# CPJKU/audio_sheet_retrieval

Hardware: AMD Instinct MI355X
Metric: snippet-pairs/sec embedded+ranked (32-d CCA) (higher is better)
Workload: dtype f32

## Files before the change

audio_sheet_retrieval_amd/csrc/conv_wino4_kernels.hip:

```cpp
#include <hip/hip_runtime.h>
#include <stdint.h>
#include <stdlib.h>
#include <algorithm>
#include <type_traits>
#include <vector>
#include "asr_kernels.h"
#include "repack_elems.inl"
#include "wino4_epilogue.h"

#ifndef ASR_WINO4_ABL
#define ASR_WINO4_ABL 0
#endif

namespace asr {

typedef float floatx4q __attribute__((ext_vector_type(4)));
typedef float float2q __attribute__((ext_vector_type(2)));
typedef unsigned uint2q __attribute__((ext_vector_type(2)));

struct Wino4Args {
    const float *in, *wpk, *bnp;
    float *out;
    int N, H, W, OH, OW;
    int ty_img, tx_img;
    int coutp;
    int tiles;
    int total;
    double *stats;
    int epi;
};

__device__ __forceinline__ float elu_fastq(float y) { return y > 0.0f ? y : __expf(y) - 1.0f; }

__device__ __forceinline__ floatx4q bn_elu4q(floatx4q x, float mean, float scale, float beta) {
    const floatx4q y = (x - floatx4q{mean, mean, mean, mean}) * floatx4q{scale, scale, scale, scale} +
                       floatx4q{beta, beta, beta, beta};
    return floatx4q{elu_fastq(y[0]), elu_fastq(y[1]), elu_fastq(y[2]), elu_fastq(y[3])};
}
typedef int int4q __attribute__((ext_vector_type(4)));
__device__ __forceinline__ void buffer_store_q(float v, unsigned voff, int4q rsrc, unsigned soff) {
    asm volatile("buffer_store_dword %0, %1, %2, %3 offen" ::"v"(v), "v"(voff), "s"(rsrc), "s"(soff) : "memory");
}

template <typename T> __device__ __forceinline__ T splatq(float c);
template <> __device__ __forceinline__ float2q splatq<float2q>(float c) { return float2q{c, c}; }
template <> __device__ __forceinline__ floatx4q splatq<floatx4q>(float c) { return floatx4q{c, c, c, c}; }
template <typename T> __device__ __forceinline__ T fmaq(float c, T x, T y) {
    return __builtin_elementwise_fma(splatq<T>(c), x, y);
}

template <typename T> __device__ __forceinline__ void in6(T &d0, T &d1, T &d2, T &d3, T &d4, T &d5) {
    const T r0 = fmaq(4.f, d0, fmaq(-5.f, d2, d4));
    const T t1 = fmaq(-4.f, d2, d4), t2 = fmaq(-4.f, d1, d3);
    const T t3 = d4 - d2, t4 = d3 - d1;
    const T r5 = fmaq(4.f, d1, fmaq(-5.f, d3, d5));
    d0 = r0; d1 = t1 + t2; d2 = t1 - t2; d3 = fmaq(2.f, t4, t3); d4 = fmaq(-2.f, t4, t3); d5 = r5;
}
template <typename T> __device__ __forceinline__ void out6(T m0, T m1, T m2, T m3, T m4, T m5, T &y0, T &y1, T &y2, T &y3) {
    const T s1 = m1 + m2, s2 = m1 - m2, s3 = m3 + m4, s4 = m3 - m4;
    y0 = (m0 + s1) + s3;
    y1 = fmaq(2.f, s4, s2);
    y2 = fmaq(4.f, s3, s1);
    y3 = fmaq(8.f, s4, s2) + m5;
}

template <int CIN, int COUT, bool POOL, int WAVES, bool RAW>
__global__ __launch_bounds__(64 * WAVES, 1) void conv3x3_wino4g(Wino4Args a) {
    constexpr int KS = CIN / 4, NB = CIN / 8, T = 64 * WAVES;
    constexpr int WS = 16;
    constexpr int WD = 6;
    constexpr int WQ = 72;
    static_assert(CIN % 8 == 0, "channel blocks of 8");
    extern __shared__ __align__(16) float w_lds[];
    const int tid = threadIdx.x, lane = tid & 63;
    const int wave = __builtin_amdgcn_readfirstlane(tid >> 6);
    const int nt0 = blockIdx.y;
    for (int i = tid; i < KS * 36 * 4 * 16; i += T) {
        const int row = i >> 4, nn = i & 15;
        const int gg = row & 3, kp = row >> 2, ks = kp / 36, p = kp - ks * 36;
        const int qq = (ks & 1) * 36 + p;
        w_lds[i] = a.wpk[((((size_t)(ks >> 1) * 18 + (qq >> 2)) * 4 + gg) * a.coutp + nt0 * 16 + nn) * 4 + (qq & 3)];
    }
    __syncthreads();

    const int m = lane & 15, g = lane >> 4, n = lane & 15;
    const float *w_lane = w_lds + g * WS + n;
    const int chn = nt0 * 16 + n;
    const bool ch_ok = chn < COUT;
    const float bmean = (!RAW && ch_ok) ? a.bnp[chn] : 0.f;
    const float bscale = (!RAW && ch_ok) ? a.bnp[a.coutp + chn] : 1.f;
    const float bbeta = (!RAW && ch_ok) ? a.bnp[2 * a.coutp + chn] : 0.f;
    const int per_img = a.ty_img * a.tx_img;

    for (int mt = blockIdx.x * WAVES + wave; mt < a.total; mt += gridDim.x * WAVES) {
        const int tnum = mt * 16 + m;
        const bool tvalid = tnum < a.tiles;
        const int tcl = min(tnum, a.tiles - 1);
        const int img = tcl / per_img;
        const int trest = tcl - img * per_img;
        const int tty = trest / a.tx_img, ttx = trest - tty * a.tx_img;
        const int py = 4 * tty, px = 4 * ttx;
        const float *ibase = a.in + (int64_t)img * a.H * a.W * CIN + 2 * g;
        int rowb[6], colb[6];
        unsigned oy_m = 0, ox_m = 0;
#pragma unroll
        for (int i = 0; i < 6; ++i) {
            const int y = py - 1 + i, x = px - 1 + i;
            oy_m |= (unsigned)(y >= 0 && y < a.H) << i;
            ox_m |= (unsigned)(x >= 0 && x < a.W) << i;
            rowb[i] = min(max(y, 0), a.H - 1) * a.W * CIN;
            colb[i] = min(max(x, 0), a.W - 1) * CIN;
        }
        if (!tvalid) oy_m = 0;
        const bool interior = __builtin_amdgcn_ballot_w64(oy_m != 0x3fu || ox_m != 0x3fu) == 0;
        unsigned my_off;
        int my_ext;
        if (POOL) {
            my_off = (((unsigned)img * a.OH + 2 * tty) * a.OW + 2 * ttx) * COUT;
            const int nr = min(2, a.OH - 2 * tty), nc = min(2, a.OW - 2 * ttx);
            my_ext = (tvalid && nr > 0 && nc > 0) ? (nr | (nc << 8)) : 0;
        } else {
            my_off = (((unsigned)img * a.H + py) * a.W + px) * COUT;
            const int nr = min(4, a.H - py), nc = min(4, a.W - px);
            my_ext = tvalid ? (nr | (nc << 8)) : 0;
        }

        floatx4q acc[36];
#pragma unroll
        for (int p = 0; p < 36; ++p) acc[p] = floatx4q{0.f, 0.f, 0.f, 0.f};

        float2q nxt[6][6];
#pragma unroll
        for (int i = 0; i < 6; ++i)
#pragma unroll
            for (int j = 0; j < 6; ++j) nxt[i][j] = *reinterpret_cast<const float2q *>(ibase + rowb[i] + colb[j]);
        float wpre[WD];
#pragma unroll
        for (int q = 0; q < WD; ++q) wpre[q] = w_lane[q * 4 * WS];
#pragma unroll 1
        for (int t = 0; t < NB; ++t) {
            float2q dp[6][6];
            if (interior) {
#pragma unroll
                for (int i = 0; i < 6; ++i)
#pragma unroll
                    for (int j = 0; j < 6; ++j) dp[i][j] = nxt[i][j];
            } else {
#pragma unroll
                for (int i = 0; i < 6; ++i)
#pragma unroll
                    for (int j = 0; j < 6; ++j)
                        dp[i][j] = (((oy_m >> i) & (ox_m >> j)) & 1u) ? nxt[i][j] : float2q{0.f, 0.f};
            }
            if (t + 1 < NB && !(ASR_WINO4_ABL & 2)) {
#pragma unroll
                for (int i = 0; i < 6; ++i)
#pragma unroll
                    for (int j = 0; j < 6; ++j)
                        nxt[i][j] = *reinterpret_cast<const float2q *>(ibase + rowb[i] + colb[j] + 8 * (t + 1));
            }
#pragma unroll
            for (int j = 0; j < 6; ++j) in6(dp[0][j], dp[1][j], dp[2][j], dp[3][j], dp[4][j], dp[5][j]);
#pragma unroll
            for (int i = 0; i < 6; ++i) in6(dp[i][0], dp[i][1], dp[i][2], dp[i][3], dp[i][4], dp[i][5]);
            const float *wk = w_lane + (2 * t) * (36 * 4 * WS);
            const float *wn = (t + 1 < NB) ? wk + 2 * 36 * 4 * WS : w_lane;
            float wv[WQ + WD];
#pragma unroll
            for (int q = 0; q < WD; ++q) wv[q] = wpre[q];
#pragma unroll
            for (int q0 = 0; q0 < WQ; q0 += 2) {
#pragma unroll
                for (int q = q0; q < q0 + 2; ++q)
                    wv[q + WD] = (q + WD < WQ) ? wk[(q + WD) * 4 * WS] : wn[(q + WD - WQ) * 4 * WS];
                __builtin_amdgcn_sched_barrier(0);
#pragma unroll
                for (int q = q0; q < q0 + 2; ++q) {
                    const int c = q / 36, p = q % 36;
                    acc[p] = __builtin_amdgcn_mfma_f32_16x16x4f32(dp[p / 6][p % 6][c], wv[q], acc[p], 0, 0, 0);
                }
                __builtin_amdgcn_sched_barrier(0);
            }
#pragma unroll
            for (int q = 0; q < WD; ++q) wpre[q] = wv[WQ + q];
        }

        unsigned eo[4];
        int ee[4];
#pragma unroll
        for (int r = 0; r < 4; ++r) {
            eo[r] = (unsigned)__shfl((int)my_off, 4 * g + r);
            ee[r] = __shfl(my_ext, 4 * g + r);
        }
        if (!ch_ok) continue;
        floatx4q tc[4][6];
#pragma unroll
        for (int nu = 0; nu < 6; ++nu)
            out6(acc[nu], acc[6 + nu], acc[12 + nu], acc[18 + nu], acc[24 + nu], acc[30 + nu], tc[0][nu], tc[1][nu], tc[2][nu],
                 tc[3][nu]);
        if (POOL) {
#pragma unroll
            for (int pr = 0; pr < 2; ++pr) {
                floatx4q ya[4], yb[4];
                out6(tc[2 * pr][0], tc[2 * pr][1], tc[2 * pr][2], tc[2 * pr][3], tc[2 * pr][4], tc[2 * pr][5], ya[0], ya[1],
                     ya[2], ya[3]);
                out6(tc[2 * pr + 1][0], tc[2 * pr + 1][1], tc[2 * pr + 1][2], tc[2 * pr + 1][3], tc[2 * pr + 1][4],
                     tc[2 * pr + 1][5], yb[0], yb[1], yb[2], yb[3]);
#pragma unroll
                for (int pc = 0; pc < 2; ++pc) {
#pragma unroll
                    for (int r = 0; r < 4; ++r) {
                        if (pr >= (ee[r] & 0xff) || pc >= (ee[r] >> 8)) continue;
                        const float v0 = ya[2 * pc][r], v1 = ya[2 * pc + 1][r], v2 = yb[2 * pc][r], v3 = yb[2 * pc + 1][r];
                        const float hi = fmaxf(fmaxf(v0, v1), fmaxf(v2, v3));
                        const float lo = fminf(fminf(v0, v1), fminf(v2, v3));
                        const float x = bscale >= 0.0f ? hi : lo;
                        a.out[(size_t)eo[r] + (size_t)(pr * a.OW + pc) * COUT + chn] =
                            elu_fastq((x - bmean) * bscale + bbeta);
                    }
                }
            }
        } else {
#pragma unroll
            for (int i = 0; i < 4; ++i) {
                floatx4q y[4];
                out6(tc[i][0], tc[i][1], tc[i][2], tc[i][3], tc[i][4], tc[i][5], y[0], y[1], y[2], y[3]);
#pragma unroll
                for (int j = 0; j < 4; ++j) {
#pragma unroll
                    for (int r = 0; r < 4; ++r) {
                        if (i >= (ee[r] & 0xff) || j >= (ee[r] >> 8)) continue;
                        const float v = RAW ? y[j][r] : elu_fastq((y[j][r] - bmean) * bscale + bbeta);
                        a.out[(size_t)eo[r] + (size_t)(i * a.W + j) * COUT + chn] = v;
                    }
                }
            }
        }
    }
}

template <int CIN, int COUT, bool POOL, int SLICE = COUT, int PW = 1, bool RAW = false>
__global__ __launch_bounds__(64 * (PW + (SLICE + 15) / 16), 1) void conv3x3_wino4s(Wino4Args a) {
    static_assert(!(RAW && POOL), "the raw form has no pooled epilogue");
    constexpr int NT = (SLICE + 15) / 16, NB = CIN / 8, KS = CIN / 4;
    static_assert(PW == 1 || PW == 2, "one or two producer waves");
    static_assert(PW + NT <= 4, "one wave per SIMD");
    static_assert(SLICE == COUT || (SLICE % 16 == 0 && COUT % SLICE == 0), "slices are whole n-tiles");
    constexpr int VB = 36 * 16 * 8;
    static_assert(CIN % 8 == 0, "channel blocks of 8");
    extern __shared__ __align__(16) float vbuf[];
    const int tid = threadIdx.x, lane = tid & 63;
    const int wave = __builtin_amdgcn_readfirstlane(tid >> 6);
    const bool producer = wave < PW;
    const int m = lane & 15, g = lane >> 4, n = lane & 15;
    const int per_img = a.ty_img * a.tx_img;

    int mt, mt_end, mt_stride;
    if ((gridDim.x & 7) == 0) {
        const int per_x = (a.total + 7) >> 3;
        const int r0 = (int)(blockIdx.x & 7) * per_x;
        mt_end = min(r0 + per_x, a.total);
        mt_stride = (int)(gridDim.x >> 3);
        mt = r0 + (int)(blockIdx.x >> 3);
    } else {
        mt_end = a.total; mt_stride = (int)gridDim.x; mt = (int)blockIdx.x;
    }
    if (mt >= mt_end) {
        if constexpr (RAW) {
            if (a.stats)
                for (int c = threadIdx.x; c < 2 * COUT; c += blockDim.x) a.stats[(size_t)blockIdx.x * 2 * COUT + c] = 0.0;
        }
        return;
    }

    auto tile_of = [&](int mtile, int &img, int &tty, int &ttx, bool &tvalid) {
        const int tnum = mtile * 16 + m;
        tvalid = tnum < a.tiles;
        const int tcl = min(tnum, a.tiles - 1);
        img = tcl / per_img;
        const int trest = tcl - img * per_img;
        tty = trest / a.tx_img;
        ttx = trest - tty * a.tx_img;
    };
    float *vlane = vbuf + (g * 32 + 2 * m);

    if (producer) {
        unsigned poff[6][6];
        unsigned keep[6][6];
        bool interior = false;
        auto setup = [&](int mtile) {
            int img, tty, ttx;
            bool tvalid;
            tile_of(mtile, img, tty, ttx, tvalid);
            const int py = 4 * tty, px = 4 * ttx;
            const unsigned ib = ((unsigned)img * a.H * a.W * CIN + 2 * g) * 4u;
            unsigned rowb[6], colb[6];
            unsigned oy_m = 0, ox_m = 0;
#pragma unroll
            for (int i = 0; i < 6; ++i) {
                const int y = py - 1 + i, x = px - 1 + i;
                oy_m |= (unsigned)(y >= 0 && y < a.H) << i;
                ox_m |= (unsigned)(x >= 0 && x < a.W) << i;
                rowb[i] = (unsigned)(min(max(y, 0), a.H - 1) * a.W * CIN) * 4u;
                colb[i] = (unsigned)(min(max(x, 0), a.W - 1) * CIN) * 4u;
            }
            if (!tvalid) oy_m = 0;
            interior = __builtin_amdgcn_ballot_w64(oy_m != 0x3fu || ox_m != 0x3fu) == 0;
#pragma unroll
            for (int i = 0; i < 6; ++i)
#pragma unroll
                for (int j = 0; j < 6; ++j) {
                    poff[i][j] = ib + rowb[i] + colb[j];
                    keep[i][j] = 0u - (((oy_m >> i) & (ox_m >> j)) & 1u);
                }
        };
        float2q nxt[6][6];
        auto load = [&](int t) {
            const char *cb = reinterpret_cast<const char *>(a.in + 8 * t);
#pragma unroll
            for (int i = 0; i < 6; ++i)
#pragma unroll
                for (int j = 0; j < 6; ++j) nxt[i][j] = *reinterpret_cast<const float2q *>(cb + poff[i][j]);
        };
        const int n_mt = (mt_end - mt + mt_stride - 1) / mt_stride;
        const int n_steps = n_mt * NB;
        int passed = 0;
        int t = wave;
        while (t >= NB) { t -= NB; mt += mt_stride; }
        if (mt < mt_end) { setup(mt); load(t); }
        for (int step = wave; step < n_steps; step += PW) {
            constexpr int FIRST = 4;
            float2q dp[6][6];
            const bool inner = interior;
            if (inner) {
#pragma unroll
                for (int j = 0; j < 6; ++j) {
#pragma unroll
                    for (int i = 0; i < 6; ++i) dp[i][j] = nxt[i][j];
                    if (!(ASR_WINO4_ABL & 8)) in6(dp[0][j], dp[1][j], dp[2][j], dp[3][j], dp[4][j], dp[5][j]);
                }
            } else {
#pragma unroll
                for (int i = 0; i < 6; ++i)
#pragma unroll
                    for (int j = 0; j < 6; ++j)
                        dp[i][j] = __builtin_bit_cast(float2q, __builtin_bit_cast(uint2q, nxt[i][j]) & uint2q{keep[i][j], keep[i][j]});
                if (!(ASR_WINO4_ABL & 8)) {
#pragma unroll
                for (int j = 0; j < FIRST; ++j) in6(dp[0][j], dp[1][j], dp[2][j], dp[3][j], dp[4][j], dp[5][j]);
                }
            }
#pragma unroll
            for (int p = 0; p < 36; ++p) asm volatile("" : "+v"(dp[p / 6][p % 6]));
            {
                int tn = t + PW, mtn = mt;
                while (tn >= NB) { tn -= NB; mtn += mt_stride; }
                if (!(ASR_WINO4_ABL & 2) && step + PW < n_steps) {
                    if (mtn != mt) setup(mtn);
                    load(tn);
                }
                t = tn; mt = mtn;
            }
            if (!(ASR_WINO4_ABL & 8)) {
            if (!inner) {
#pragma unroll
            for (int j = FIRST; j < 6; ++j) in6(dp[0][j], dp[1][j], dp[2][j], dp[3][j], dp[4][j], dp[5][j]);
            }
#pragma unroll
            for (int i = 0; i < 6; ++i) in6(dp[i][0], dp[i][1], dp[i][2], dp[i][3], dp[i][4], dp[i][5]);
            }
            while (passed < step) { __syncthreads(); ++passed; }
            float *vb = vlane + (step & 1) * VB;
            if (!(ASR_WINO4_ABL & 16)) {
#pragma unroll
            for (int p = 0; p < 36; ++p) *reinterpret_cast<float2q *>(vb + p * 128) = dp[p / 6][p % 6];
            } else {
#pragma unroll
            for (int p = 0; p < 36; ++p) asm volatile("" ::"v"(dp[p / 6][p % 6]));
            }
            __syncthreads();
            ++passed;
        }
        while (passed < n_steps + 1) { __syncthreads(); ++passed; }
        return;
    }

    const int nt = wave - PW;
    const int chn = (int)blockIdx.y * SLICE + nt * 16 + n;
    const bool ch_ok = chn < COUT;
    float bmean = (!RAW && ch_ok) ? a.bnp[chn] : 0.f;
    float bscale = (!RAW && ch_ok) ? a.bnp[a.coutp + chn] : 1.f;
    float bbeta = (!RAW && ch_ok) ? a.bnp[2 * a.coutp + chn] : 0.f;
    double st1 = 0.0, st2 = 0.0;
    int4q orsrc;
    {
        const uint64_t obase = reinterpret_cast<uint64_t>(a.out);
        orsrc.x = (int)(uint32_t)obase;
        orsrc.y = (int)(uint32_t)(obase >> 32);
        orsrc.z = (int)((unsigned)a.N * a.OH * a.OW * COUT * 4u);
        orsrc.w = 0x00020000;
    }
    const unsigned wlane = ((unsigned)g * a.coutp + chn) * 16u;
    const float *wl = a.wpk;
    constexpr int wstep = 4 * ((COUT + 15) / 16 * 16);
    floatx4q bw[2][18];
#pragma unroll
    for (int j = 0; j < 18; ++j)
        bw[0][j] = *reinterpret_cast<const floatx4q *>(reinterpret_cast<const char *>(wl) + (size_t)j * (wstep * 16) + wlane);
    int step = 0;
    for (; mt < mt_end; mt += mt_stride) {
        unsigned my_off;
        int my_ext;
        {
            int img, tty, ttx;
            bool tvalid;
            tile_of(mt, img, tty, ttx, tvalid);
            if (POOL) my_off = (((unsigned)img * a.OH + 2 * tty) * a.OW + 2 * ttx) * COUT;
            else my_off = (((unsigned)img * a.H + 4 * tty) * a.W + 4 * ttx) * COUT;
            my_ext = wino4_extent(POOL, POOL ? a.OH : a.H, POOL ? a.OW : a.W, tty, ttx, tvalid);
        }
        int epi_mode = 0;
        if constexpr (!RAW) {
            if (a.epi)
                epi_mode = __builtin_amdgcn_ballot_w64(!wino4_rows_full(my_ext, POOL)) == 0 ? 1 : (wino4_general_form(POOL) ? 2 : 0);
        }
        unsigned voff[9];
#pragma unroll
        for (int k = 0; k < 9; ++k) {
            voff[k] = wlane + (unsigned)k * (2 * wstep * 16);
            asm volatile("" : "+v"(voff[k]));
        }
        floatx4q acc[36];
        auto reload = [&](const float *wn, auto set_c) {
            constexpr int SET = decltype(set_c)::value;
            if (ASR_WINO4_ABL & 4) return;
            const char *wnb = reinterpret_cast<const char *>(wn);
#pragma unroll
            for (int k = 0; k < 9; ++k) {
                unsigned vo = voff[k];
                asm volatile("" : "+v"(vo));
                bw[SET][2 * k] = *reinterpret_cast<const floatx4q *>(wnb + vo);
                bw[SET][2 * k + 1] = *reinterpret_cast<const floatx4q *>(wnb + (wstep * 16) + vo);
            }
        };
        auto run_step = [&](const float *vb, const float *wn, auto cur_c, auto first) {
            constexpr bool FIRST = decltype(first)::value;
            constexpr int CUR = decltype(cur_c)::value;
            using NXT = std::integral_constant<int, CUR ^ 1>;
            __syncthreads();
            reload(wn, NXT{});
            __builtin_amdgcn_sched_barrier(0);
            float2q dp[2][12];
#pragma unroll
            for (int i = 0; i < 12; ++i) dp[0][i] = *reinterpret_cast<const float2q *>(vb + i * 128);
#pragma unroll
            for (int grp = 0; grp < 3; ++grp) {
                if (grp < 2) {
#pragma unroll
                    for (int i = 0; i < 12; ++i)
                        dp[(grp + 1) & 1][i] = *reinterpret_cast<const float2q *>(vb + ((grp + 1) * 12 + i) * 128);
                }
#pragma unroll
                for (int c = 0; c < 2; ++c)
#pragma unroll
                    for (int i = 0; i < 12; ++i) {
                        const int p = grp * 12 + i;
                        if (FIRST && c == 0)
                            acc[p] = __builtin_amdgcn_mfma_f32_16x16x4f32(dp[grp & 1][i][c], bw[CUR][(c * 36 + p) >> 2][(c * 36 + p) & 3],
                                                                          floatx4q{0.f, 0.f, 0.f, 0.f}, 0, 0, 0);
                        else
                            acc[p] = __builtin_amdgcn_mfma_f32_16x16x4f32(dp[grp & 1][i][c], bw[CUR][(c * 36 + p) >> 2][(c * 36 + p) & 3], acc[p],
                                                                          0, 0,
                                                                          0);
                    }
                __builtin_amdgcn_sched_barrier(0);
            }
        };
        using C0 = std::integral_constant<int, 0>;
        using C1 = std::integral_constant<int, 1>;
        auto wblock = [&](int t) {
            unsigned blk = (unsigned)(((t + 1) % NB) * 72) * wstep;
            asm volatile("" : "+s"(blk));
            return wl + blk;
        };
        run_step(vlane + (step & 1) * VB, wblock(0), C0{}, std::true_type{});
        ++step;
#pragma unroll 1
        for (int t = 1; t + 1 < NB; t += 2) {
            run_step(vlane + (step & 1) * VB, wblock(t), C1{}, std::false_type{});
            ++step;
            run_step(vlane + (step & 1) * VB, wblock(t + 1), C0{}, std::false_type{});
            ++step;
        }
        if constexpr ((NB & 1) == 0) {
            run_step(vlane + (step & 1) * VB, wblock(NB - 1), C1{}, std::false_type{});
            ++step;
        } else {
#pragma unroll
            for (int j = 0; j < 18; ++j) bw[0][j] = bw[1][j];
        }

        unsigned eo[4];
        int ee[4];
#pragma unroll
        for (int r = 0; r < 4; ++r) {
            eo[r] = (unsigned)__shfl((int)my_off, 4 * g + r);
            ee[r] = __shfl(my_ext, 4 * g + r);
        }
        if (!ch_ok) continue;
        floatx4q tc[4][6];
#pragma unroll
        for (int nu = 0; nu < 6; ++nu)
            out6(acc[nu], acc[6 + nu], acc[12 + nu], acc[18 + nu], acc[24 + nu], acc[30 + nu], tc[0][nu], tc[1][nu], tc[2][nu],
                 tc[3][nu]);
        auto fast_epilogue = [&](auto rows_c) {
            constexpr bool ROWS = decltype(rows_c)::value;
            constexpr int SP = POOL ? 2 : 4;
            unsigned vo[4][SP];
#pragma unroll
            for (int r = 0; r < 4; ++r)
#pragma unroll
                for (int c = 0; c < SP; ++c) vo[r][c] = wino4_store_offset(eo[r], ee[r], chn, c, COUT);
#pragma unroll
            for (int i = 0; i < SP; ++i) {
                const unsigned soff = wino4_row_bytes(i, a.OW, COUT);
                floatx4q res[SP];
                if constexpr (POOL) {
                    floatx4q ya[4], yb[4];
                    out6(tc[2 * i][0], tc[2 * i][1], tc[2 * i][2], tc[2 * i][3], tc[2 * i][4], tc[2 * i][5], ya[0], ya[1], ya[2],
                         ya[3]);
                    out6(tc[2 * i + 1][0], tc[2 * i + 1][1], tc[2 * i + 1][2], tc[2 * i + 1][3], tc[2 * i + 1][4],
                         tc[2 * i + 1][5], yb[0], yb[1], yb[2], yb[3]);
#pragma unroll
                    for (int pc = 0; pc < 2; ++pc) {
                        const floatx4q hi = __builtin_elementwise_max(__builtin_elementwise_max(ya[2 * pc], ya[2 * pc + 1]),
                                                                      __builtin_elementwise_max(yb[2 * pc], yb[2 * pc + 1]));
                        const floatx4q lo = __builtin_elementwise_min(__builtin_elementwise_min(ya[2 * pc], ya[2 * pc + 1]),
                                                                      __builtin_elementwise_min(yb[2 * pc], yb[2 * pc + 1]));
                        res[pc] = bn_elu4q(bscale >= 0.0f ? hi : lo, bmean, bscale, bbeta);
                    }
                } else {
                    floatx4q y[4];
                    out6(tc[i][0], tc[i][1], tc[i][2], tc[i][3], tc[i][4], tc[i][5], y[0], y[1], y[2], y[3]);
#pragma unroll
                    for (int j = 0; j < 4; ++j) res[j] = bn_elu4q(y[j], bmean, bscale, bbeta);
                }
#pragma unroll
                for (int j = 0; j < SP; ++j)
#pragma unroll
                    for (int r = 0; r < 4; ++r) {
                        if (ASR_WINO4_ABL & 32) asm volatile("" ::"v"(res[j][r]));
                        else buffer_store_q(res[j][r], ROWS ? wino4_store_offset_row(vo[r][j], ee[r], i) : vo[r][j], orsrc, soff);
                    }
            }
        };
        if (epi_mode == 1) { fast_epilogue(std::false_type{}); continue; }
        if constexpr (!RAW && wino4_general_form(POOL)) {
            if (epi_mode == 2) { fast_epilogue(std::true_type{}); continue; }
        }
        if (POOL) {
#pragma unroll
            for (int pr = 0; pr < 2; ++pr) {
                floatx4q ya[4], yb[4];
                out6(tc[2 * pr][0], tc[2 * pr][1], tc[2 * pr][2], tc[2 * pr][3], tc[2 * pr][4], tc[2 * pr][5], ya[0], ya[1],
                     ya[2], ya[3]);
                out6(tc[2 * pr + 1][0], tc[2 * pr + 1][1], tc[2 * pr + 1][2], tc[2 * pr + 1][3], tc[2 * pr + 1][4],
                     tc[2 * pr + 1][5], yb[0], yb[1], yb[2], yb[3]);
#pragma unroll
                for (int pc = 0; pc < 2; ++pc) {
#pragma unroll
                    for (int r = 0; r < 4; ++r) {
                        if (pr >= (ee[r] & 0xff) || pc >= (ee[r] >> 8)) continue;
                        const float v0 = ya[2 * pc][r], v1 = ya[2 * pc + 1][r], v2 = yb[2 * pc][r], v3 = yb[2 * pc + 1][r];
                        const float hi = fmaxf(fmaxf(v0, v1), fmaxf(v2, v3));
                        const float lo = fminf(fminf(v0, v1), fminf(v2, v3));
                        const float x = bscale >= 0.0f ? hi : lo;
                        const float res = elu_fastq((x - bmean) * bscale + bbeta);
                        if (ASR_WINO4_ABL & 32) asm volatile("" ::"v"(res));
                        else a.out[(size_t)eo[r] + (size_t)(pr * a.OW + pc) * COUT + chn] = res;
                    }
                }
            }
        } else {
#pragma unroll
            for (int i = 0; i < 4; ++i) {
                floatx4q y[4];
                out6(tc[i][0], tc[i][1], tc[i][2], tc[i][3], tc[i][4], tc[i][5], y[0], y[1], y[2], y[3]);
                float rs1 = 0.f, rs2 = 0.f;
#pragma unroll
                for (int j = 0; j < 4; ++j) {
#pragma unroll
                    for (int r = 0; r < 4; ++r) {
                        if (i >= (ee[r] & 0xff) || j >= (ee[r] >> 8)) continue;
                        const float res = RAW ? y[j][r] : elu_fastq((y[j][r] - bmean) * bscale + bbeta);
                        if (RAW) { rs1 += res; rs2 = fmaf(res, res, rs2); }
                        if (ASR_WINO4_ABL & 32) asm volatile("" ::"v"(res));
                        else a.out[(size_t)eo[r] + (size_t)(i * a.W + j) * COUT + chn] = res;
                    }
                }
                if (RAW) { st1 += (double)rs1; st2 += (double)rs2; }
            }
        }
    }
    __syncthreads();
    if constexpr (RAW) {
        if (a.stats) {
            st1 += __shfl_xor(st1, 16); st2 += __shfl_xor(st2, 16);
            st1 += __shfl_xor(st1, 32); st2 += __shfl_xor(st2, 32);
            if (g == 0 && ch_ok) {
                a.stats[((size_t)blockIdx.x * 2) * COUT + chn] = st1;
                a.stats[((size_t)blockIdx.x * 2 + 1) * COUT + chn] = st2;
            }
        }
    }
}

__global__ void wino4_pack_kernel(const float *W, int cin, int cout, int dgrad, float *wpk) {
    const int idx = blockIdx.x * blockDim.x + threadIdx.x;
    if (idx >= wino4_pack_count(cin, cout, dgrad)) return;
    wino4_pack_elem(idx, W, cin, cout, dgrad, wpk);
}

size_t wino4_wpack_floats(int cin, int cout) { return (cin % 8) ? 0 : (size_t)36 * cin * ((cout + 15) / 16 * 16); }

hipError_t launch_wino4_pack(hipStream_t s, const float *W, int cin, int cout, float *wpk, int dgrad) {
    const int kdim = dgrad ? cout : cin, ndim = dgrad ? cin : cout;
    if (kdim % 8) return hipSuccess;
    const int total = kdim * ((ndim + 15) / 16 * 16);
    hipLaunchKernelGGL(wino4_pack_kernel, dim3((total + 255) / 256), dim3(256), 0, s, W, cin, cout, dgrad, wpk);
    return hipGetLastError();
}

struct Wino4Variant {
    int cin, cout, pool, waves, raw;
    void (*kernel)(Wino4Args);
    const char *symbol;
    int spec;
    int slice;
};
#define ASR_BOOLSTRQ_0 "false"
#define ASR_BOOLSTRQ_1 "true"
#define ASR_WINO4(CIN, COUT, POOL, WAVES)                                                                         \
    { CIN, COUT, POOL, WAVES, 0, conv3x3_wino4g<CIN, COUT, (POOL != 0), WAVES, false>,                            \
      "void asr::conv3x3_wino4g<" #CIN ", " #COUT ", " ASR_BOOLSTRQ_##POOL ", " #WAVES ", false>(asr::Wino4Args)" }
#define ASR_WINO4S(CIN, COUT, POOL)                                                                               \
    { CIN, COUT, POOL, 1 + (COUT + 15) / 16, 0, conv3x3_wino4s<CIN, COUT, (POOL != 0)>,                           \
      "void asr::conv3x3_wino4s<" #CIN ", " #COUT ", " ASR_BOOLSTRQ_##POOL ", " #COUT ", 1, false>(asr::Wino4Args)", 1, 0 }
#define ASR_WINO4S2(CIN, COUT, POOL)                                                                              \
    { CIN, COUT, POOL, 2 + (COUT + 15) / 16, 0, conv3x3_wino4s<CIN, COUT, (POOL != 0), COUT, 2>,                  \
      "void asr::conv3x3_wino4s<" #CIN ", " #COUT ", " ASR_BOOLSTRQ_##POOL ", " #COUT ", 2, false>(asr::Wino4Args)", 1, 0 }
#define ASR_WINO4SR(CIN, COUT)                                                                                    \
    { CIN, COUT, 0, 1 + (COUT + 15) / 16, 1, conv3x3_wino4s<CIN, COUT, false, COUT, 1, true>,                     \
      "void asr::conv3x3_wino4s<" #CIN ", " #COUT ", false, " #COUT ", 1, true>(asr::Wino4Args)", 1, 0 }
#define ASR_WINO4SL(CIN, COUT, POOL, SLICE)                                                                       \
    { CIN, COUT, POOL, 1 + SLICE / 16, 0, conv3x3_wino4s<CIN, COUT, (POOL != 0), SLICE>,                          \
      "void asr::conv3x3_wino4s<" #CIN ", " #COUT ", " ASR_BOOLSTRQ_##POOL ", " #SLICE ", 1, false>(asr::Wino4Args)", 1, SLICE }
static const Wino4Variant g_wino4[] = {
    ASR_WINO4(24, 24, 1, 4), ASR_WINO4(24, 48, 0, 4), ASR_WINO4(48, 48, 1, 4), ASR_WINO4(48, 48, 0, 4),
    ASR_WINO4S(24, 24, 1), ASR_WINO4S(24, 48, 0), ASR_WINO4S(48, 48, 1), ASR_WINO4S(48, 48, 0),
    ASR_WINO4S2(24, 24, 1),
    ASR_WINO4SL(48, 96, 0, 48), ASR_WINO4SL(96, 96, 1, 48), ASR_WINO4SL(96, 96, 0, 48),
    ASR_WINO4SR(24, 48), ASR_WINO4SR(48, 48), ASR_WINO4SR(48, 24),
};
static const int g_num_wino4 = (int)(sizeof(g_wino4) / sizeof(g_wino4[0]));

void conv_candidates_wino4(int cin, int cout, int pool, int H, int W, std::vector<ConvPlan> *out) {
    static const int use = getenv("ASR_CONV_WINO4") ? atoi(getenv("ASR_CONV_WINO4")) : -1;
    if (use == 0) return;
    const int epi = getenv("ASR_WINO4_EPI") ? (atoi(getenv("ASR_WINO4_EPI")) != 0) : 1;
    for (int vi = 0; vi < g_num_wino4; ++vi) {
        const Wino4Variant &v = g_wino4[vi];
        if (v.cin != cin || v.cout != cout || v.pool != pool || v.raw) continue;
        if (!v.spec && use != 1) continue;
        const int lds = v.spec ? 2 * 36 * 16 * 8 * 4 : 36 * cin * 16 * 4;
        (void)hipFuncSetAttribute(reinterpret_cast<const void *>(v.kernel), hipFuncAttributeMaxDynamicSharedMemorySize,
                                  160 * 1024);
        int nb = 0;
        if (hipOccupancyMaxActiveBlocksPerMultiprocessor(&nb, reinterpret_cast<const void *>(v.kernel), 64 * v.waves,
                                                         (size_t)lds) != hipSuccess || nb < 1) {
            (void)hipGetLastError();
            nb = 1;
        }
        ConvPlan bp{};
        bp.cin = cin; bp.cout = cout; bp.pool = pool;
        bp.H = H; bp.W = W; bp.OH = pool ? H / 2 : H; bp.OW = pool ? W / 2 : W;
        bp.TH = 4; bp.TW = 64; bp.NI = 16;
        bp.tiles_y = ((pool ? 2 * bp.OH : H) + 3) / 4; bp.tiles_x = ((pool ? 2 * bp.OW : W) + 3) / 4;
        bp.threads = 64 * v.waves;
        bp.lds_bytes = lds;
        bp.blocks_per_cu = v.spec ? 1 : std::min(nb, 4);
        bp.cost = (double)bp.tiles_y * bp.tiles_x / 16.0 * ((cout + 15) / 16) * (36.0 * (cin / 4) * 32.0 + 3000.0) *
                  (v.spec ? 0.4 : 1.0);
        bp.variant = 4000 + vi;
        bp.symbol = v.symbol;
        bp.epi = v.spec ? epi : 0;
        out->push_back(bp);
    }
}

void conv_candidates_wino4_raw(int cin, int cout, int H, int W, std::vector<ConvPlan> *out, int dgrad) {
    static const int use = getenv("ASR_TRAIN_WINO4") ? atoi(getenv("ASR_TRAIN_WINO4")) : -1;
    if (use == 0 || (use == 5 && !dgrad)) return;
    for (int vi = 0; vi < g_num_wino4; ++vi) {
        const Wino4Variant &v = g_wino4[vi];
        if (v.cin != cin || v.cout != cout || !v.raw) continue;
        const int lds = 2 * 36 * 16 * 8 * 4;
        (void)hipFuncSetAttribute(reinterpret_cast<const void *>(v.kernel), hipFuncAttributeMaxDynamicSharedMemorySize,
                                  160 * 1024);
        ConvPlan bp{};
        bp.cin = cin; bp.cout = cout; bp.pool = 0;
        bp.H = H; bp.W = W; bp.OH = H; bp.OW = W;
        bp.TH = 4; bp.TW = 64; bp.NI = 16;
        bp.tiles_y = (H + 3) / 4; bp.tiles_x = (W + 3) / 4;
        bp.threads = 64 * v.waves;
        bp.lds_bytes = lds;
        bp.blocks_per_cu = 1;
        bp.cost = (double)bp.tiles_y * bp.tiles_x / 16.0 * ((cout + 15) / 16) * (36.0 * (cin / 4) * 32.0 + 3000.0) * 0.4;
        bp.variant = 4000 + vi;
        bp.symbol = v.symbol;
        out->push_back(bp);
    }
}
bool conv_wino4_is_raw(const ConvPlan &p) { return p.variant >= 4000 && g_wino4[p.variant - 4000].raw != 0; }
int conv_wino4_stats_rows_max(int num_cus) { return num_cus; }

static int wino4_grid(const ConvPlan &p, const Wino4Variant &v, int total, int num_cus, int *groups_out) {
    if (v.spec) {
        const int slices = v.slice ? p.cout / v.slice : 1;
        int grid = std::min(total, std::max(1, num_cus * std::max(1, p.blocks_per_cu) / slices));
        if (grid >= 8) grid &= ~7;
        *groups_out = slices;
        return grid;
    }
    const int ntiles = (p.cout + 15) / 16;
    const int waves = p.threads / 64;
    const int slots = std::max(1, num_cus * std::max(1, p.blocks_per_cu) / ntiles);
    *groups_out = ntiles;
    return std::min((total + waves - 1) / waves, slots);
}

void conv_wino4_launch_shape(const ConvPlan &p, int N, int num_cus, int *items, int *grid_x) {
    int groups = 0;
    *items = (N * p.tiles_y * p.tiles_x + 15) / 16;
    *grid_x = *items ? wino4_grid(p, g_wino4[p.variant - 4000], *items, num_cus, &groups) : 0;
}

hipError_t launch_conv_wino4(hipStream_t s, const ConvPlan &p, const float *in, const float *wpk, const float *bnp,
                             float *out, int N, int num_cus, double *stats, int *stats_rows) {
    const Wino4Variant &v = g_wino4[p.variant - 4000];
    Wino4Args a;
    a.epi = (p.epi && v.spec && !v.raw && wino4_fast_epilogue_admitted(N, p.OH, p.OW, p.cout)) ? 1 : 0;
    a.stats = nullptr;
    a.in = in; a.wpk = wpk; a.bnp = bnp; a.out = out;
    a.N = N; a.H = p.H; a.W = p.W; a.OH = p.OH; a.OW = p.OW;
    a.ty_img = p.tiles_y; a.tx_img = p.tiles_x;
    a.coutp = (p.cout + 15) / 16 * 16;
    a.tiles = N * a.ty_img * a.tx_img;
    a.total = (a.tiles + 15) / 16;
    if (a.total == 0) return hipSuccess;
    if (v.spec) {
        if ((double)N * p.H * p.W * p.cin * 4.0 >= 4294967296.0) return hipErrorInvalidValue;
        int slices = 0;
        const int grid = wino4_grid(p, v, a.total, num_cus, &slices);
        if (v.raw && stats) {
            a.stats = stats;
            if (stats_rows) *stats_rows = grid;
        }
        hipLaunchKernelGGL(v.kernel, dim3(grid, slices), dim3(p.threads), p.lds_bytes, s, a);
        return hipGetLastError();
    }
    int ntiles = 0;
    const int grid = wino4_grid(p, v, a.total, num_cus, &ntiles);
    hipLaunchKernelGGL(v.kernel, dim3(grid, ntiles), dim3(p.threads), p.lds_bytes, s, a);
    return hipGetLastError();
}

}
```

Measured before the change: 319,800.

## Hold Winograd weights in AGPRs with inline-asm MFMA and explicit vmcnt waits

```diff
diff --git a/audio_sheet_retrieval_amd/csrc/conv_wino4_kernels.hip b/audio_sheet_retrieval_amd/csrc/conv_wino4_kernels.hip
--- a/audio_sheet_retrieval_amd/csrc/conv_wino4_kernels.hip
+++ b/audio_sheet_retrieval_amd/csrc/conv_wino4_kernels.hip
@@ -40,6 +40,32 @@
 typedef int int4q __attribute__((ext_vector_type(4)));
 __device__ __forceinline__ void buffer_store_q(float v, unsigned voff, int4q rsrc, unsigned soff) {
     asm volatile("buffer_store_dword %0, %1, %2, %3 offen" ::"v"(v), "v"(voff), "s"(rsrc), "s"(soff) : "memory");
+}
+
+__device__ __forceinline__ floatx4q wino4_load_weights(const char *base, unsigned voff) {
+    floatx4q d;
+    asm volatile("global_load_dwordx4 %0, %1, %2" : "=a"(d) : "v"(voff), "s"(base));
+    return d;
+}
+template <int N> __device__ __forceinline__ void wino4_wait_weights(floatx4q *w) {
+    static_assert(N >= 0 && N <= 63, "vmcnt is a 6-bit field");
+    asm volatile("s_waitcnt vmcnt(%18)"
+                 : "+a"(w[0]), "+a"(w[1]), "+a"(w[2]), "+a"(w[3]), "+a"(w[4]), "+a"(w[5]), "+a"(w[6]), "+a"(w[7]), "+a"(w[8]),
+                   "+a"(w[9]), "+a"(w[10]), "+a"(w[11]), "+a"(w[12]), "+a"(w[13]), "+a"(w[14]), "+a"(w[15]), "+a"(w[16]),
+                   "+a"(w[17])
+                 : "n"(N));
+}
+__device__ __forceinline__ void wino4_mfma(floatx4q &acc, float a, float b) {
+    asm volatile("v_mfma_f32_16x16x4_f32 %0, %1, %2, %0" : "+v"(acc) : "v"(a), "a"(b));
+}
+__device__ __forceinline__ void wino4_mfma_zero(floatx4q &acc, float a, float b) {
+    asm volatile("v_mfma_f32_16x16x4_f32 %0, %1, %2, 0" : "=&v"(acc) : "v"(a), "a"(b));
+}
+__device__ __forceinline__ void wino4_settle(floatx4q *c) {
+    asm volatile("s_nop 15"
+                 : "+v"(c[0]), "+v"(c[1]), "+v"(c[2]), "+v"(c[3]), "+v"(c[4]), "+v"(c[5]), "+v"(c[6]), "+v"(c[7]), "+v"(c[8]),
+                   "+v"(c[9]), "+v"(c[10]), "+v"(c[11]), "+v"(c[12]), "+v"(c[13]), "+v"(c[14]), "+v"(c[15]), "+v"(c[16]),
+                   "+v"(c[17]));
 }
 
 template <typename T> __device__ __forceinline__ T splatq(float c);
@@ -403,10 +429,25 @@
     const unsigned wlane = ((unsigned)g * a.coutp + chn) * 16u;
     const float *wl = a.wpk;
     constexpr int wstep = 4 * ((COUT + 15) / 16 * 16);
-    floatx4q bw[2][18];
-#pragma unroll
-    for (int j = 0; j < 18; ++j)
-        bw[0][j] = *reinterpret_cast<const floatx4q *>(reinterpret_cast<const char *>(wl) + (size_t)j * (wstep * 16) + wlane);
+    constexpr bool RESIDENT = !RAW && CIN == 24;
+    static_assert(RAW || RESIDENT || (NB & 1) == 0, "the streamed sets alternate over an even number of steps");
+    constexpr int NSETS = RESIDENT ? NB : 2;
+    floatx4q bw[NSETS * 18];
+    if constexpr (RAW) {
+#pragma unroll
+        for (int j = 0; j < 18; ++j)
+            bw[j] = *reinterpret_cast<const floatx4q *>(reinterpret_cast<const char *>(wl) + (size_t)j * (wstep * 16) + wlane);
+    } else {
+#pragma unroll
+        for (int j = 0; j < (RESIDENT ? NSETS : 1) * 18; ++j)
+            bw[j] = wino4_load_weights(reinterpret_cast<const char *>(wl) + (size_t)j * (wstep * 16), wlane);
+        if constexpr (RESIDENT) {
+#pragma unroll
+            for (int s = 0; s < NSETS; ++s) wino4_wait_weights<0>(bw + 18 * s);
+        }
+    }
+    constexpr int FAST_STORES = POOL ? 16 : 64;
+    bool after_fast = false;
     int step = 0;
     for (; mt < mt_end; mt += mt_stride) {
         unsigned my_off;
@@ -425,10 +466,12 @@
                 epi_mode = __builtin_amdgcn_ballot_w64(!wino4_rows_full(my_ext, POOL)) == 0 ? 1 : (wino4_general_form(POOL) ? 2 : 0);
         }
         unsigned voff[9];
-#pragma unroll
-        for (int k = 0; k < 9; ++k) {
-            voff[k] = wlane + (unsigned)k * (2 * wstep * 16);
-            asm volatile("" : "+v"(voff[k]));
+        if constexpr (!RESIDENT) {
+#pragma unroll
+            for (int k = 0; k < 9; ++k) {
+                voff[k] = wlane + (unsigned)k * (2 * wstep * 16);
+                asm volatile("" : "+v"(voff[k]));
+            }
         }
         floatx4q acc[36];
         auto reload = [&](const float *wn, auto set_c) {
@@ -437,18 +480,25 @@
             const char *wnb = reinterpret_cast<const char *>(wn);
 #pragma unroll
             for (int k = 0; k < 9; ++k) {
-                unsigned vo = voff[k];
-                asm volatile("" : "+v"(vo));
-                bw[SET][2 * k] = *reinterpret_cast<const floatx4q *>(wnb + vo);
-                bw[SET][2 * k + 1] = *reinterpret_cast<const floatx4q *>(wnb + (wstep * 16) + vo);
+                if constexpr (RAW) {
+                    unsigned vo = voff[k];
+                    asm volatile("" : "+v"(vo));
+                    bw[18 * SET + 2 * k] = *reinterpret_cast<const floatx4q *>(wnb + vo);
+                    bw[18 * SET + 2 * k + 1] = *reinterpret_cast<const floatx4q *>(wnb + (wstep * 16) + vo);
+                } else {
+                    bw[18 * SET + 2 * k] = wino4_load_weights(wnb, voff[k]);
+                    bw[18 * SET + 2 * k + 1] = wino4_load_weights(wnb + (wstep * 16), voff[k]);
+                }
             }
         };
-        auto run_step = [&](const float *vb, const float *wn, auto cur_c, auto first) {
+        auto run_step = [&](const float *vb, const float *wn, auto cur_c, auto first, auto wait_c) {
             constexpr bool FIRST = decltype(first)::value;
             constexpr int CUR = decltype(cur_c)::value;
-            using NXT = std::integral_constant<int, CUR ^ 1>;
             __syncthreads();
-            reload(wn, NXT{});
+            if constexpr (!RESIDENT) {
+                reload(wn, std::integral_constant<int, CUR ^ 1>{});
+                if constexpr (!RAW) wino4_wait_weights<decltype(wait_c)::value>(bw + 18 * CUR);
+            }
             __builtin_amdgcn_sched_barrier(0);
             float2q dp[2][12];
 #pragma unroll
@@ -460,44 +510,69 @@
                     for (int i = 0; i < 12; ++i)
                         dp[(grp + 1) & 1][i] = *reinterpret_cast<const float2q *>(vb + ((grp + 1) * 12 + i) * 128);
                 }
+                if constexpr (!RAW) asm volatile("s_nop 1");
 #pragma unroll
                 for (int c = 0; c < 2; ++c)
 #pragma unroll
                     for (int i = 0; i < 12; ++i) {
                         const int p = grp * 12 + i;
-                        if (FIRST && c == 0)
-                            acc[p] = __builtin_amdgcn_mfma_f32_16x16x4f32(dp[grp & 1][i][c], bw[CUR][(c * 36 + p) >> 2][(c * 36 + p) & 3],
-                                                                          floatx4q{0.f, 0.f, 0.f, 0.f}, 0, 0, 0);
-                        else
-                            acc[p] = __builtin_amdgcn_mfma_f32_16x16x4f32(dp[grp & 1][i][c], bw[CUR][(c * 36 + p) >> 2][(c * 36 + p) & 3], acc[p],
-                                                                          0, 0,
-                                                                          0);
+                        const int q = c * 36 + p;
+                        if constexpr (RAW) {
+                            if (FIRST && c == 0)
+                                acc[p] = __builtin_amdgcn_mfma_f32_16x16x4f32(dp[grp & 1][i][c], bw[18 * CUR + (q >> 2)][q & 3],
+                                                                              floatx4q{0.f, 0.f, 0.f, 0.f}, 0, 0, 0);
+                            else
+                                acc[p] = __builtin_amdgcn_mfma_f32_16x16x4f32(dp[grp & 1][i][c], bw[18 * CUR + (q >> 2)][q & 3], acc[p],
+                                                                              0, 0, 0);
+                        } else {
+                            if (FIRST && c == 0) wino4_mfma_zero(acc[p], dp[grp & 1][i][c], bw[18 * CUR + (q >> 2)][q & 3]);
+                            else wino4_mfma(acc[p], dp[grp & 1][i][c], bw[18 * CUR + (q >> 2)][q & 3]);
+                        }
                     }
                 __builtin_amdgcn_sched_barrier(0);
             }
         };
         using C0 = std::integral_constant<int, 0>;
         using C1 = std::integral_constant<int, 1>;
+        using C2 = std::integral_constant<int, 2>;
+        using W18 = std::integral_constant<int, 18>;
+        using WFAST = std::integral_constant<int, (18 + FAST_STORES < 63 ? 18 + FAST_STORES : 63)>;
         auto wblock = [&](int t) {
             unsigned blk = (unsigned)(((t + 1) % NB) * 72) * wstep;
             asm volatile("" : "+s"(blk));
             return wl + blk;
         };
-        run_step(vlane + (step & 1) * VB, wblock(0), C0{}, std::true_type{});
-        ++step;
-#pragma unroll 1
-        for (int t = 1; t + 1 < NB; t += 2) {
-            run_step(vlane + (step & 1) * VB, wblock(t), C1{}, std::false_type{});
+        if constexpr (RESIDENT) {
+            static_assert(!RESIDENT || NB == 3, "one step per resident set");
+            run_step(vlane + (step & 1) * VB, wl, C0{}, std::true_type{}, W18{});
             ++step;
-            run_step(vlane + (step & 1) * VB, wblock(t + 1), C0{}, std::false_type{});
+            run_step(vlane + (step & 1) * VB, wl, C1{}, std::false_type{}, W18{});
             ++step;
-        }
-        if constexpr ((NB & 1) == 0) {
-            run_step(vlane + (step & 1) * VB, wblock(NB - 1), C1{}, std::false_type{});
+            run_step(vlane + (step & 1) * VB, wl, C2{}, std::false_type{}, W18{});
             ++step;
         } else {
-#pragma unroll
-            for (int j = 0; j < 18; ++j) bw[0][j] = bw[1][j];
+            if (!RAW && after_fast) run_step(vlane + (step & 1) * VB, wblock(0), C0{}, std::true_type{}, WFAST{});
+            else run_step(vlane + (step & 1) * VB, wblock(0), C0{}, std::true_type{}, W18{});
+            after_fast = false;
+            ++step;
+#pragma unroll 1
+            for (int t = 1; t + 1 < NB; t += 2) {
+                run_step(vlane + (step & 1) * VB, wblock(t), C1{}, std::false_type{}, W18{});
+                ++step;
+                run_step(vlane + (step & 1) * VB, wblock(t + 1), C0{}, std::false_type{}, W18{});
+                ++step;
+            }
+            if constexpr ((NB & 1) == 0) {
+                run_step(vlane + (step & 1) * VB, wblock(NB - 1), C1{}, std::false_type{}, W18{});
+                ++step;
+            } else {
+#pragma unroll
+                for (int j = 0; j < 18; ++j) bw[j] = bw[18 + j];
+            }
+        }
+        if constexpr (!RAW) {
+            wino4_settle(acc);
+            wino4_settle(acc + 18);
         }
 
         unsigned eo[4];
@@ -554,9 +629,9 @@
                     }
             }
         };
-        if (epi_mode == 1) { fast_epilogue(std::false_type{}); continue; }
+        if (epi_mode == 1) { fast_epilogue(std::false_type{}); after_fast = !(ASR_WINO4_ABL & 32); continue; }
         if constexpr (!RAW && wino4_general_form(POOL)) {
-            if (epi_mode == 2) { fast_epilogue(std::true_type{}); continue; }
+            if (epi_mode == 2) { fast_epilogue(std::true_type{}); after_fast = !(ASR_WINO4_ABL & 32); continue; }
         }
         if (POOL) {
 #pragma unroll
```

New measurement: 325,800, median of 6. 1.02x the previous value.
